# philips/janus

Hardware: AMD Instinct MI355X
Metric: reports prepared+aggregated/sec (helper, Prio3Histogram len=256) at 1/2/4/8 GPUs (higher is better)
Workload: dtype u32 limbs (Field128 mod-p integer arithmetic); 1 GPU; Prio3Histogram length=256 chunk_length=16 helper prepare_init+prepare_shares_to_prepare_message+prepare_next+aggregate, 1 segment; reports_per_gpu=1048576, global_batch=1048576, parallelism=dp1 (report shards; RCCL all-gather + mod-p combine)

## Files before the change

### include/janus_prio3.h

```cpp
#ifndef JANUS_PRIO3_H
#define JANUS_PRIO3_H
#include <stddef.h>
#include <stdint.h>

#ifdef __cplusplus
extern "C" {
#endif

enum {
  PRIO3_COUNT = 0,
  PRIO3_SUM = 1,
  PRIO3_SUMVEC = 2,
  PRIO3_HISTOGRAM = 3,
  PRIO3_SUMVEC_F64_MP = 4,
  PRIO3_FPVEC_BOUNDED_L2 = 5,
};

enum {
  PRIO3_STATUS_FINISHED = 0,
  PRIO3_STATUS_PREP_INIT = 1,
  PRIO3_STATUS_PREP_SHARE_DECODE = 2,
  PRIO3_STATUS_PREP_MSG = 3,
  PRIO3_STATUS_PREP_NEXT = 4,
  PRIO3_STATUS_PEER_MISMATCH = 5,
// ... 170 lines not shown
                             uint8_t* status);

struct janus_hpke_sealer;
int prio3_client_report_stride(const prio3_params* params,
                               const struct janus_hpke_sealer* leader_sealer,
                               const struct janus_hpke_sealer* helper_sealer,
                               int with_taskprov_extension);
int prio3_client_prepare_reports_device(
    prio3_engine* engine, struct janus_hpke_sealer* leader_sealer,
    struct janus_hpke_sealer* helper_sealer, uint32_t n, const uint8_t task_id[32],
    uint64_t time_precision, const uint64_t* d_measurements, const uint8_t* d_report_ids,
    const uint64_t* d_times, const uint8_t* d_rand, const uint8_t* d_sk_e_leader,
    const uint8_t* d_sk_e_helper, uint8_t leader_config_id, uint8_t helper_config_id,
    int with_taskprov_extension, uint8_t* d_reports, uint32_t report_stride,
    uint32_t* d_report_len, uint8_t* d_status, void* stream);

int prio3_client_generate_device(prio3_engine* engine, uint32_t n, uint64_t seed,
                                 uint64_t first_index, uint8_t* d_nonces,
                                 uint8_t* d_public_shares, uint8_t* d_helper_shares,
                                 uint8_t* d_leader_prep_shares, uint64_t* d_measurements,
                                 uint8_t* d_leader_out_shares, uint8_t* d_flags,
                                 uint8_t* d_leader_input_shares, void* stream);

int prio3_device_trim(int device);

int prio3_engine_set_option(prio3_engine* engine, const char* key, int64_t value);
int prio3_engine_timing(prio3_engine* engine, char* names, size_t names_cap, double* ms,
                        uint64_t* launches, int cap);
void prio3_engine_timing_reset(prio3_engine* engine);
int prio3_trace_enabled(void);

int prio3_selftest_field(int op, uint32_t n, const uint8_t* a, const uint8_t* b, uint8_t* out);

#ifdef __cplusplus
}
#endif
#endif
```

### janus_amd/csrc/prio3_device.h

```cpp
#pragma once
#include <hip/hip_runtime.h>
#include <stdint.h>

#define DEV __device__ __forceinline__
#ifndef F128_ASM
#define F128_ASM 1
#endif

struct f128 {
  uint32_t w[4];
};

DEV f128 mk128(uint32_t a, uint32_t b, uint32_t c, uint32_t d) {
  f128 r;
  r.w[0] = a;
  r.w[1] = b;
  r.w[2] = c;
  r.w[3] = d;
  return r;
}
DEV f128 zero128() { return mk128(0, 0, 0, 0); }
DEV f128 sel128(bool c, const f128& a, const f128& b) {
  return mk128(c ? a.w[0] : b.w[0], c ? a.w[1] : b.w[1], c ? a.w[2] : b.w[2], c ? a.w[3] : b.w[3]);
}
// ... 639 lines not shown
#pragma unroll
  for (int i = 0; i < N / 2; i++) {
    const uint32_t lo = v[i], hi = v[i + N / 2];
    const uint32_t send = sel ? lo : hi, keep = sel ? hi : lo;
    v[i] = keep + (uint32_t)__builtin_amdgcn_update_dpp(0, (int)send, CTRL, 0xf, 0xf, false);
  }
}
DEV uint32_t wave_halfsum2(const f128& x0, const f128& x1, uint32_t lane) {
  uint32_t v[16];
#pragma unroll
  for (int w = 0; w < 4; w++) {
    v[2 * w] = x0.w[w] & 0xffffu;
    v[2 * w + 1] = x0.w[w] >> 16;
    v[8 + 2 * w] = x1.w[w] & 0xffffu;
    v[8 + 2 * w + 1] = x1.w[w] >> 16;
  }
#pragma unroll
  for (int i = 0; i < 8; i++) {
    const auto r = __builtin_amdgcn_permlane32_swap(v[i], v[i + 8], false, false);
    v[i] = r[0] + r[1];
  }
#pragma unroll
  for (int i = 0; i < 4; i++) {
    const auto r = __builtin_amdgcn_permlane16_swap(v[i], v[i + 4], false, false);
    v[i] = r[0] + r[1];
  }
  halfsum_stage<4, 0x140, 3>(v, lane);
  halfsum_stage<2, 0x141, 2>(v, lane);
  uint32_t x = v[0];
  x += (uint32_t)__builtin_amdgcn_update_dpp(0, (int)x, 0xB1, 0xf, 0xf, false);
  x += (uint32_t)__builtin_amdgcn_update_dpp(0, (int)x, 0x4E, 0xf, 0xf, false);
  return x;
}
```

### janus_amd/csrc/prio3_engine.hip

```cpp
#include <hip/hip_runtime.h>

#include <cstdio>
#include <cstdlib>
#include <cstring>
#include <functional>
#include <mutex>
#include <string>
#include <thread>
#include <type_traits>
#include <vector>

#include "../../include/janus_hpke.h"
#include "../../include/janus_prio3.h"
#include "prio3_device.h"

#include "prio3_common.h"
#include "prio3_query_sum.h"
#include "prio3_runtime.h"
#include "sha256_device.h"
#include "sha256_host.h"

#ifndef XOFD_OCC
#define XOFD_OCC 3
#endif
template <class F>
__device__ __forceinline__ void xof_body(const DevParams& p, const InPtrs& in, const Scratch& sc,
                                         const uint32_t r) {
  if (r >= p.n) return;
  constexpr uint32_t ES = F::ES;
  uint32_t flag = p.force_slow;
  uint32_t nonce[4], km[4], kp[4], kb[4] = {0, 0, 0, 0};
  load16(in.nonces + 16 * (size_t)r, nonce);
  const uint8_t* hs = in.helper + (size_t)r * p.helper_share_len;
  load16(hs, km);
  load16(hs + 16, kp);
  const bool JR = p.jr_len > 0;
  if (JR) load16(hs + 32, kb);

  {
    KState s;
    kzero(s);
    Msg m;
    msg_zero(m);
    msg_dst(m, p.dst[5]);
    {
      uint32_t vk[4];
      load_vk(p, in, r, vk);
      msg_bytes16(m, 9, vk);
    }
    msg_byte(m, 25, 1);
    msg_bytes16(m, 26, nonce);
    msg_absorb_final(s, m, 42);
    uint32_t q0 = 0, q1 = 0;
    squeeze_block<F>(p, s, 0, p.qr_len, q0, q1, sc.qr, r, flag);
// ... 168 lines not shown
    msg_dst(m, p.dst[5]);
    {
      uint32_t vk[4];
      load_vk(p, in, r, vk);
      msg_bytes16(m, 9, vk);
    }
    msg_byte(m, 25, 1);
    msg_bytes16(m, 26, nonce);
    msg_absorb_final(s, m, 42);
    if (p.qr_len == 1) {
      uint32_t w[4] = {kword(s, 0), kword(s, 1), kword(s, 2), kword(s, 3)};
      put_elem<F>(p, sc.qr, 0, r, w, flag);
    } else {
      uint32_t q0 = 0, q1 = 0;
      squeeze_block<F>(p, s, 0, p.qr_len, q0, q1, sc.qr, r, flag);
    }
  }
  const uint32_t M = p.meas_len, K = (M * 16 + 167) / 168;
  const uint32_t L = 42 + M * 16, B = L / 168, rem = L % 168;
  KState ms, js;
  kzero(ms);
  kzero(js);
  {
    Msg m;
    msg_zero(m);
    msg_dst(m, p.dst[1]);
    msg_bytes16(m, 9, km);
    msg_byte(m, 25, 1);
    msg_absorb_final(ms, m, 26);
  }
  uint32_t pend0 = 0, pend1 = 0;
  TruncSink ts(p, sc.out, r);
  const int Mi = (int)M;
  auto fused_pair = [&](int e0, f128 a, f128 b2) __attribute__((always_inline)) {
    if (e0 >= Mi) return;
    if (haspad && oor) {
      a = zero128();
      b2 = zero128();
    }
    const uint32_t tot = wave_halfsum2(a, b2, lane);
    const int e = e0 + (int)(lane >> 5);
    if ((lane & 3u) == 0 && e < Mi)
      sc.wpart[((size_t)(r >> 6) * M + (uint32_t)e) * 8u + ((lane >> 2) & 7u)] = tot;
  };
  auto fuse_block = [&](uint32_t b, uint32_t q0, uint32_t q1) __attribute__((always_inline)) {
    const int e0 = 21 * (int)(b >> 1);
    const f128 z = zero128();
    if ((b & 1) == 0) {
#pragma unroll
      for (int t = 0; t < 10; t += 2)
        fused_pair(e0 + t, mk128(kword(ms, 4 * t), kword(ms, 4 * t + 1), kword(ms, 4 * t + 2),
                                 kword(ms, 4 * t + 3)),
                   mk128(kword(ms, 4 * t + 4), kword(ms, 4 * t + 5), kword(ms, 4 * t + 6),
                         kword(ms, 4 * t + 7)));
    } else {
      fused_pair(e0 + 10, mk128(q0, q1, kword(ms, 0), kword(ms, 1)),
                 mk128(kword(ms, 2), kword(ms, 3), kword(ms, 4), kword(ms, 5)));
#pragma unroll
      for (int t = 1; t < 10; t += 2)
        fused_pair(e0 + 11 + t,
                   mk128(kword(ms, 2 + 4 * t), kword(ms, 3 + 4 * t), kword(ms, 4 + 4 * t),
                         kword(ms, 5 + 4 * t)),
                   t + 1 < 10 ? mk128(kword(ms, 6 + 4 * t), kword(ms, 7 + 4 * t),
                                      kword(ms, 8 + 4 * t), kword(ms, 9 + 4 * t))
                              : z);
    }
  };
  auto wmask = [&](int j) __attribute__((always_inline)) {
    const uint32_t lo = 4u * (uint32_t)j;
    return (lo + 4 <= rem) ? 0xffffffffu : (lo >= rem ? 0u : ((1u << (8 * (rem - lo))) - 1u));
  };
  auto carry_tail = [&](bool last) __attribute__((always_inline)) {
#pragma unroll
    for (int j = 0; j < 10; j++) {
      uint32_t x = __builtin_amdgcn_alignbit(kword(ms, 32 + j), kword(ms, 31 + j), 16);
      if (last) x &= wmask(j);
      kxor_word(js, j, x);
    }
    uint32_t x = kword(ms, 41) >> 16;
    if (last) x &= wmask(10);
    kxor_word(js, 10, x);
  };
  {
    if (FUSE && fuse) fuse_block(0, 0, 0);
    squeeze_meas<TR>(p, ms, 0, M, pend0, pend1, sc.meas, r, flag, ts);
    Msg m;
    msg_zero(m);
    msg_dst(m, p.dst[7]);
    msg_bytes16(m, 9, kb);
    msg_byte(m, 25, 1);
    msg_bytes16(m, 26, nonce);
#pragma unroll
    for (int j = 0; j < 10; j++) kxor_word(js, j, m.w[j]);
    kxor_word(js, 10, (m.w[10] & 0xffffu) | (kword(ms, 0) << 16));
#pragma unroll
    for (int j = 11; j < 42; j++)
      kxor_word(js, j, __builtin_amdgcn_alignbit(kword(ms, j - 10), kword(ms, j - 11), 16));
    keccak_p12(js);
    carry_tail(B == 1);
    keccak_p12(ms);
  }
  if constexpr (PULL) {
    if (in.seg_dst) in.seg_dst[r] = in.seg_src[r];
    if (in.accept_dst) in.accept_dst[r] = in.accept_src[r];
  }
  const uint32_t Q = PULL ? p.prep_share_len / 16 : 0u;
  const size_t wbase = PULL ? (size_t)(r - lane) * (p.prep_share_len / 16) + lane : 0;
  const uint4* lsrc = PULL ? (const uint4*)in.leader_src + wbase : nullptr;
  uint4* ldst = PULL ? (uint4*)in.leader + wbase : nullptr;
#pragma unroll 1
  for (uint32_t b = 1; b < B; b++) {
    uint4 pc0, pc1;
    uint32_t q0 = 0, q1 = 0;
    if constexpr (PULL) {
      q0 = Q * (b - 1) / (B - 1);
      q1 = Q * b / (B - 1);
      if (q0 < q1) pc0 = lsrc[64 * (size_t)q0];
      if (q0 + 1 < q1) pc1 = lsrc[64 * (size_t)(q0 + 1)];
    }
    if (FUSE && fuse) fuse_block(b, pend0, pend1);
    squeeze_meas<TR>(p, ms, b, M, pend0, pend1, sc.meas, r, flag, ts);
    kxor_word(js, 10, kword(ms, 0) << 16);
#pragma unroll
    for (int j = 11; j < 42; j++)
      kxor_word(js, j, __builtin_amdgcn_alignbit(kword(ms, j - 10), kword(ms, j - 11), 16));
    keccak_p12(js);
    carry_tail(b + 1 == B);
    if (b + 1 < K) keccak_p12(ms);
    if constexpr (PULL) {
      if (q0 < q1) ldst[64 * (size_t)q0] = pc0;
      if (q0 + 1 < q1) ldst[64 * (size_t)(q0 + 1)] = pc1;
    }
  }
  uint32_t part[4];
  {
    const bool hasW = B < K;
    if (FUSE && fuse && hasW) fuse_block(B, pend0, pend1);
    if (hasW) squeeze_meas<TR>(p, ms, B, M, pend0, pend1, sc.meas, r, flag, ts);
#pragma unroll
    for (int j = 0; j < 42; j++) {
      uint32_t x = 0;
      if (j == 10) x = hasW ? kword(ms, 0) << 16 : 0u;
      else if (j > 10)
        x = hasW ? __builtin_amdgcn_alignbit(kword(ms, j - 10), kword(ms, j - 11), 16) : 0u;
      x &= wmask(j);
      if ((uint32_t)j == (rem >> 2)) x ^= 1u << (8 * (rem & 3));
      if (j == 41) x ^= 0x80000000u;
      kxor_word(js, j, x);
    }
    keccak_p12(js);
    part[0] = kword(js, 0);
    part[1] = kword(js, 1);
    part[2] = kword(js, 2);
    part[3] = kword(js, 3);
  }
  {
    uint32_t kp[4];
    load16(hs + 16, kp);
    KState s;
    kzero(s);
    Msg m;
    msg_zero(m);
    msg_dst(m, p.dst[2]);
    msg_bytes16(m, 9, kp);
    msg_byte(m, 25, 1);
    msg_byte(m, 26, 1);
    msg_absorb_final(s, m, 27);
    const uint32_t PL = p.proof_len, Kp = (PL * 16 + 167) / 168;
    uint32_t q0 = 0, q1 = 0;
    for (uint32_t b = 0; b < Kp; b++) {
      squeeze_block<F>(p, s, b, PL, q0, q1, sc.proofs, r, flag);
      if (b + 1 < Kp) keccak_p12(s);
    }
  }
  {
    uint32_t pub0[4];
    load16(in.pub + (size_t)r * p.public_share_len, pub0);
    KState s;
    kzero(s);
    Msg m;
    msg_zero(m);
    msg_dst(m, p.dst[6]);
    msg_bytes16(m, 25, pub0);
    msg_bytes16(m, 41, part);
    msg_absorb_final(s, m, 57);
    uint32_t cor[4] = {kword(s, 0), kword(s, 1), kword(s, 2), kword(s, 3)};
    KState t;
    kzero(t);
    Msg m2;
    msg_zero(m2);
    msg_dst(m2, p.dst[3]);
    msg_bytes16(m2, 9, cor);
    msg_byte(m2, 25, 1);
    msg_absorb_final(t, m2, 26);
    uint32_t q0 = 0, q1 = 0;
    squeeze_block<F>(p, t, 0, p.jr_len, q0, q1, sc.jr, r, flag);
    sc.part[r] = make_uint4(part[0], part[1], part[2], part[3]);
    sc.corrected[r] = make_uint4(cor[0], cor[1], cor[2], cor[3]);
  }
  sc.flag[r] = (uint8_t)flag;
  if constexpr (FUSE) {
    if (fuse) {
      const bool anyflag = __any(flag != 0);
      if (lane == 0) sc.wseg[r >> 6] = anyflag ? 0xffffffffu : s0;
    }
  }
}
template <bool FUSE, bool TR = false>
__global__ __launch_bounds__(256, XOFD_OCC) void k_xofd(DevParams p, InPtrs in, Scratch sc) {
  xofd_body<FUSE, TR>(p, in, sc, blockIdx.x * blockDim.x + threadIdx.x);
}

struct ZeroRanges {
  uint8_t* dst[4];
  size_t bytes[4];
};
__global__ __launch_bounds__(256) void k_zero(ZeroRanges z) {
  const size_t tid = blockIdx.x * (size_t)blockDim.x + threadIdx.x, nth = (size_t)gridDim.x * blockDim.x;
#pragma unroll
  for (int k = 0; k < 4; k++) {
    uint8_t* d = z.dst[k];
    const size_t n = z.bytes[k];
    if (!d || !n) continue;
    const size_t head = std::min(n, (size_t)((16 - ((uintptr_t)d & 15)) & 15));
    const size_t n16 = (n - head) / 16;
    for (size_t i = tid; i < n16; i += nth) ((uint4*)(d + head))[i] = make_uint4(0, 0, 0, 0);
    for (size_t i = tid * 4; i < head; i += nth * 4) *(uint32_t*)(d + i) = 0u;
    for (size_t i = head + 16 * n16 + tid * 4; i < n; i += nth * 4) *(uint32_t*)(d + i) = 0u;
  }
}

struct PullRanges {
  const uint8_t* src[4];
  uint8_t* dst[4];
  size_t bytes[4];
};
DEV void pull_body(const PullRanges& pr, size_t tid, size_t nth) {
#pragma unroll
  for (int k = 0; k < 4; k++) {
    const size_t n16 = pr.bytes[k] / 16;
    const uint4* s16 = (const uint4*)pr.src[k];
    uint4* d16 = (uint4*)pr.dst[k];
// ... 1175 lines not shown
  const T PT = F::add(lv(A + 1), pt);
  if (status == PRIO3_STATUS_FINISHED) {
    if (!decode_ok)
      status = PRIO3_STATUS_PREP_SHARE_DECODE;
    else if (!F::is_zero(V0) || !F::eq(G, PT))
      status = PRIO3_STATUS_PREP_MSG;
  }
  uint32_t lpart[4], msg[4];
  load16(lps + (size_t)p.verifier_len * F::ES, lpart);
  if (!prep_msg_check(p, in, sc, r, lpart, msg) && status == PRIO3_STATUS_FINISHED)
    status = PRIO3_STATUS_PREP_NEXT;
  if (status != PRIO3_STATUS_FINISHED) msg[0] = msg[1] = msg[2] = msg[3] = 0;
  ((uint4*)out.prep_msgs)[r] = make_uint4(msg[0], msg[1], msg[2], msg[3]);
  out.status[r] = status;
  }
  if (p.kind == PRIO3_SUMVEC) {
    for (uint32_t e = 0; e < p.out_len; e++) {
      T acc = F::zero(), pw = F::one();
      for (uint32_t b = 0; b < p.bits; b++) {
        acc = F::add(acc, F::mul(pw, ldf<F>(sc.meas, e * p.bits + b, ld, r)));
        pw = F::add(pw, pw);
      }
      F::store(sc.out, (size_t)e * ld + r, acc);
    }
  }
}
template <int GS, int PP, int LEADER = 0>
__global__ __launch_bounds__(256, 3) void k_query_h(DevParams p, InPtrs in, Scratch sc,
                                                  OutPtrs out) {
  query_h_body<GS, PP, LEADER>(p, in, sc, out, blockIdx.x * blockDim.x + threadIdx.x);
}

template <bool FUSE, bool PULL = false>
__global__ __launch_bounds__(256, 3) void k_prep_h(DevParams p, InPtrs in, Scratch sc,
                                                   OutPtrs out) {
  const uint32_t r = blockIdx.x * blockDim.x + threadIdx.x;
  xofd_body<FUSE, false, PULL>(p, in, sc, r);
  query_h_body<2, 32>(p, in, sc, out, r);
}

template <int PP>
__global__ __launch_bounds__(256, 3) void k_leader_prep(DevParams p, InPtrs in, Scratch sc,
                                                        OutPtrs out, uint32_t* wpart,
                                                        uint32_t* wseg) {
  const uint32_t r = blockIdx.x * blockDim.x + threadIdx.x;
  leader_jr_body(p, in, sc, out.status, wpart, wseg, r);
  query_h_body<2, PP, 1>(p, in, sc, out, r);
}

template <int NPH>
__global__ __launch_bounds__(256, 3) void k_prep_sum(DevParams p, InPtrs in, Scratch sc,
                                                     OutPtrs out) {
  const uint32_t r = blockIdx.x * blockDim.x + threadIdx.x;
  xofd_body<false, false>(p, in, sc, r);
  qsum::query_sum_body<NPH, 0>(p, in, sc, out, r);
}





template <class F, int SG>
__global__ __launch_bounds__(256) void k_acc_seg(uint32_t n, size_t ld, uint32_t chunk,
                                                 uint32_t out_len, uint32_t nseg, const void* src,
                                                 const uint8_t* status, const uint32_t* seg,
                                                 const uint8_t* accept, void* partial,
                                                 uint64_t* pcount) {
// ... 534 lines not shown
    iv_out[2 * s] = hi ? lo : 0;
    iv_out[2 * s + 1] = hi ? hi - lo : 0;
  }
}

__global__ void k_meta_final(uint32_t n_segments, unsigned long long* iv) {
  const uint32_t s = blockIdx.x * blockDim.x + threadIdx.x;
  if (s >= n_segments) return;
  const unsigned long long lo = iv[2 * s], hi = iv[2 * s + 1];
  iv[2 * s] = hi ? lo : 0;
  iv[2 * s + 1] = hi ? hi - lo : 0;
}


__global__ void k_selftest_f128(int op, uint32_t n, const uint4* a, const uint4* b, uint4* out) {
  const uint32_t i = blockIdx.x * blockDim.x + threadIdx.x;
  if (i >= n) return;
  auto ld = [](const uint4* p, size_t k) {
    const uint4 v = p[k];
    return mk128(v.x, v.y, v.z, v.w);
  };
  f128 z;
  if (op == 0) z = mul128(ld(a, i), ld(b, i));
  else if (op == 1) z = mul128_asm(ld(a, i), ld(b, i));
  else if (op == 2) z = add128(ld(a, i), ld(b, i));
  else if (op == 3) z = sub128(ld(a, i), ld(b, i));
  else {
    mac128 m;
    mac_zero(m);
    for (int k = 0; k < 16; k++) mac_add(m, ld(a, (size_t)i * 16 + k), ld(b, (size_t)i * 16 + k));
    z = op == 4 ? mac_reduce(m) : mac_reduce_asm(m);
  }
  out[i] = make_uint4(z.w[0], z.w[1], z.w[2], z.w[3]);
}




struct prio3_batch {
  prio3_engine* e;
  Run* run;
  uint32_t c0, n;
};

static uint32_t next_pow2(uint32_t n) {
  uint32_t p = 1;
  while (p < n) p <<= 1;
  return p;
}

static uint32_t optimal_chunk_length(uint32_t m) {
  if (m <= 1) return 1;
  uint32_t max_log2 = 0;
  while ((1u << max_log2) < m) max_log2++;
  max_log2 += 1;
  uint64_t best = UINT64_MAX;
  uint32_t best_chunk = 1;
  for (uint32_t l = max_log2; l >= 1; l--) {
    const uint64_t calls = (1ull << l) - 1, chunk = (m + calls - 1) / calls;
    const uint64_t cost = 2 * chunk + 2 * ((1ull << l) - 1) + 1;
    if (cost < best) {
      best = cost;
      best_chunk = (uint32_t)chunk;
    }
  }
  return best_chunk;
// ... 531 lines not shown
  const bool dual = dp.es == 16 && dp.jr_len && (42 + dp.meas_len * 16) / 168 >= 2;
  if (dp.kind == PRIO3_SUM) return dual && !fuse && query_sum_takes(dp);
  return ps && dual && dp.P == 32;
}

enum : int { DEFER_NONE = 0, DEFER_QH = 1, DEFER_SUM = 2, DEFER_GEN64 = 3 };
static int launch_prepare(prio3_engine* e, const DevParams& base, uint32_t c0, uint32_t n,
                          InPtrs in, OutPtrs out, Scratch sc, hipStream_t st, bool fuse,
                          int* deferred, bool pair = false) {
  DevParams dp = base;
  dp.n = n;
  dp.force_slow = (uint32_t)e->force_slow;
  dp.slow_defer = 0;
  dp.redo = 0;
  const size_t es = dp.es;
  in.nonces += 16 * (size_t)c0;
  if (in.pub) in.pub += (size_t)dp.public_share_len * c0;
  in.helper += (size_t)dp.helper_share_len * c0;
  in.leader += (size_t)dp.prep_share_len * c0;
  if (in.vk_slot) in.vk_slot += c0;
  out.prep_msgs += (size_t)(dp.kind == PRIO3_SUMVEC_F64_MP ? 32 : 16) * c0;
  out.status += c0;
  void** soa[] = {&sc.meas, &sc.proofs, &sc.jr, &sc.qr, &sc.Lbuf, &sc.PVbuf, &sc.acc, &sc.out,
                  &sc.beta};
  for (auto q : soa)
    if (*q) *q = (uint8_t*)*q + es * c0;
  sc.part += c0;
  sc.corrected += c0;
  sc.flag += c0;
  if (sc.seg) sc.seg += c0;
  if (sc.wseg) sc.wseg += c0 / 64;
  if (sc.wpart) sc.wpart += (size_t)(c0 / 64) * dp.meas_len * 8;
  const uint32_t blocks = (n + 255) / 256;
  if (dp.kind == PRIO3_SUMVEC_F64_MP) {
    int rc = PRIO3_OK;
    TIMED(e, st, "k_mp64_prepare", (rc = launch_mp64(e, n, dp.ld, in, out, sc, st)));
    return rc;
  }
  if (dp.kind == PRIO3_FPVEC_BOUNDED_L2) {
    uint32_t nsub, sub;
    const bool qwide = !e->force_generic && fpvec_query_wide_takes(dp);
    fp_sub_sizes(e, n, dp.ld, qwide, nsub, sub);
    for (uint32_t si = 0; si < nsub; si++) {
      const uint32_t s0 = si * sub;
      DevParams q = dp;
      q.n = si + 1 < nsub ? sub : n - s0;
      InPtrs qi = in;
      qi.nonces += 16 * (size_t)s0;
      qi.pub += (size_t)dp.public_share_len * s0;
      qi.helper += (size_t)dp.helper_share_len * s0;
      qi.leader += (size_t)dp.prep_share_len * s0;
      if (qi.vk_slot) qi.vk_slot += s0;
      OutPtrs qo = out;
      qo.prep_msgs += 16 * (size_t)s0;
      qo.status += s0;
      Scratch qs = sc;
      qs.out = (uint8_t*)sc.out + es * s0;
      const uint32_t qb = (q.n + 255) / 256;
      const bool dual = (42 + dp.meas_len * 16) / 168 >= 2;
      q.trunc_xof = dual ? 1u : 0u;
      bool paired = false;
      if (dual) TIMED(e, st, "k_xof_pair", (paired = launch_xof_pair(q, qi, qs, st)));
      if (!paired && dual)
        TIMED(e, st, "k_xofd", (k_xofd<false, true><<<qb, 256, 0, st>>>(q, qi, qs)));
      else if (!paired)
        TIMED(e, st, "k_xof", (k_xof<Fp128><<<qb, 256, 0, st>>>(q, qi, qs)));
      TIMED(e, st, "k_xof_slow", launch_xof_slow<Fp128>(e, q, qi, qs, st));
      if (qwide)
        TIMED(e, st, "k_query_fpw", launch_fpvec_query(q, qi, qs, qo, st, true, false));
      else
        TIMED(e, st, "k_query_fp", launch_fpvec_query(q, qi, qs, qo, st, false, false));
    }
    return PRIO3_OK;
  }
  if (dp.es == 16) {
    const bool ps = dp.kind == PRIO3_HISTOGRAM || dp.kind == PRIO3_SUMVEC;
    const bool wide = ps && !e->force_generic && dp.P != 32 && query_wide_takes(dp);
    const bool dual = dp.jr_len && (42 + dp.meas_len * 16) / 168 >= 2;
    dp.trunc_xof = dp.kind == PRIO3_SUMVEC && wide && dual && !fuse ? 1u : 0u;
    if (prep_fused_takes(e, dp, fuse)) {
      dp.slow_defer = 1u;
      if (dp.kind == PRIO3_SUM) {
        if (deferred) *deferred = DEFER_SUM;
        switch (dp.P) {
          case 16: TIMED(e, st, "k_prep_sum", (k_prep_sum<1><<<blocks, 256, 0, st>>>(dp, in, sc, out))); break;
          case 32: TIMED(e, st, "k_prep_sum", (k_prep_sum<2><<<blocks, 256, 0, st>>>(dp, in, sc, out))); break;
          case 64: TIMED(e, st, "k_prep_sum", (k_prep_sum<4><<<blocks, 256, 0, st>>>(dp, in, sc, out))); break;
          default: TIMED(e, st, "k_prep_sum", (k_prep_sum<8><<<blocks, 256, 0, st>>>(dp, in, sc, out))); break;
        }
      } else {
        if (deferred) *deferred = DEFER_QH;
        const bool pl = in.leader_src != nullptr;
        bool paired = false;
        if (pair)
          TIMED(e, st, "k_prep_hp", (paired = launch_prep_pair(dp, in, sc, out, st, fuse, pl)));
        if (paired) {
        } else if (fuse && pl)
          TIMED(e, st, "k_prep_h", (k_prep_h<true, true><<<blocks, 256, 0, st>>>(dp, in, sc, out)));
        else if (fuse)
          TIMED(e, st, "k_prep_h", (k_prep_h<true><<<blocks, 256, 0, st>>>(dp, in, sc, out)));
        else if (pl)
          TIMED(e, st, "k_prep_h", (k_prep_h<false, true><<<blocks, 256, 0, st>>>(dp, in, sc, out)));
        else
          TIMED(e, st, "k_prep_h", (k_prep_h<false><<<blocks, 256, 0, st>>>(dp, in, sc, out)));
      }
      return PRIO3_OK;
    }
    if (dual) {
      if (fuse)
        TIMED(e, st, "k_xofd", (k_xofd<true><<<blocks, 256, 0, st>>>(dp, in, sc)));
      else if (dp.trunc_xof)
        TIMED(e, st, "k_xofd", (k_xofd<false, true><<<blocks, 256, 0, st>>>(dp, in, sc)));
      else
        TIMED(e, st, "k_xofd", (k_xofd<false><<<blocks, 256, 0, st>>>(dp, in, sc)));
    } else {
      TIMED(e, st, "k_xof_a", (k_xof_a<Fp128><<<blocks, 256, 0, st>>>(dp, in, sc)));
      TIMED(e, st, "k_jrpart", (k_jrpart<false><<<blocks, 256, 0, st>>>(dp, in, sc)));
    }
    const bool qh_path =
        ps && !e->force_generic && !wide && (dp.P == 32 || dp.P == 16 || dp.P == 8);
    dp.slow_defer = qh_path ? 1u : 0u;
    if (qh_path && deferred) *deferred = DEFER_QH;
    if (!qh_path) TIMED(e, st, "k_xof_slow", launch_xof_slow<Fp128>(e, dp, in, sc, st));
    bool done = false;
    if (wide) TIMED(e, st, "k_query_w", (done = launch_query_wide(dp, in, sc, out, st)));
    if (done) {
    } else if (qh_path && dp.P == 32)
      TIMED(e, st, "k_query_h", (k_query_h<2, 32><<<blocks, 256, 0, st>>>(dp, in, sc, out)));
    else if (qh_path && dp.P == 16)
      TIMED(e, st, "k_query_h", (k_query_h<2, 16><<<blocks, 256, 0, st>>>(dp, in, sc, out)));
    else if (qh_path && dp.P == 8)
      TIMED(e, st, "k_query_h", (k_query_h<2, 8><<<blocks, 256, 0, st>>>(dp, in, sc, out)));
    else if (ps)
      TIMED(e, st, "k_query_ps", (k_query_ps<4><<<blocks, 256, 0, st>>>(dp, in, sc, out)));
    else {
      bool qs = false;
      if (!e->force_generic && query_sum_takes(dp))
        TIMED(e, st, "k_query_sum", (qs = launch_query_sum(dp, in, sc, out, st)));
      if (!qs) TIMED(e, st, "k_query", (k_query<Fp128><<<blocks, 256, 0, st>>>(dp, in, sc, out)));
    }
  } else {
    dp.slow_defer = 1u;
    if (deferred) *deferred = DEFER_GEN64;
    TIMED(e, st, "k_prep_gen", (k_prep_gen<Fp64><<<blocks, 256, 0, st>>>(dp, in, sc, out)));
  }
  return PRIO3_OK;
}
// ... 1954 lines not shown
    return exec_leader_next(&job);
  }
  int rc = prio3_leader_prepare_next_batch(b, prep_msgs, status_inout);
  if (rc == PRIO3_OK)
    rc = prio3_accumulate(b, segment_ids, accept_mask, n_segments, agg_shares_out, counts_out);
  return rc;
}

int prio3_trace_enabled(void) { return trace_enabled() ? 1 : 0; }

int prio3_selftest_field(int op, uint32_t n, const uint8_t* a, const uint8_t* b, uint8_t* out) {
  if (op < 0 || op > 5) return PRIO3_EINVAL;
  if (n == 0) return PRIO3_OK;
  const size_t m = (op >= 4 ? 16 : 1) * (size_t)n * 16;
  void *da = nullptr, *db = nullptr, *dout = nullptr;
  int rc = PRIO3_OK;
  if (hipMalloc(&da, m) != hipSuccess || hipMalloc(&db, m) != hipSuccess ||
      hipMalloc(&dout, (size_t)n * 16) != hipSuccess ||
      hipMemcpy(da, a, m, hipMemcpyHostToDevice) != hipSuccess ||
      hipMemcpy(db, b, m, hipMemcpyHostToDevice) != hipSuccess) {
    rc = PRIO3_EDEVICE;
  } else {
    k_selftest_f128<<<(n + 255) / 256, 256>>>(op, n, (const uint4*)da, (const uint4*)db, (uint4*)dout);
    if (hipGetLastError() != hipSuccess ||
        hipMemcpy(out, dout, (size_t)n * 16, hipMemcpyDeviceToHost) != hipSuccess)
      rc = PRIO3_EDEVICE;
  }
  (void)hipFree(da);
  (void)hipFree(db);
  (void)hipFree(dout);
  return rc;
}

}
```

### janus_amd/prio3.py

```python
from __future__ import annotations

import ctypes as C
import os
from dataclasses import dataclass
from typing import Optional

import numpy as np

_HERE = os.path.dirname(os.path.abspath(__file__))
LIB_PATH = os.environ.get("JANUS_PRIO3_LIB") or os.path.join(_HERE, "libjanus_prio3.so")

PRIO3_COUNT, PRIO3_SUM, PRIO3_SUMVEC, PRIO3_HISTOGRAM, PRIO3_SUMVEC_F64_MP = 0, 1, 2, 3, 4
PRIO3_FPVEC_BOUNDED_L2 = 5

STATUS_FINISHED = 0
STATUS_PREP_INIT = 1
STATUS_PREP_SHARE_DECODE = 2
STATUS_PREP_MSG = 3
STATUS_PREP_NEXT = 4
STATUS_PEER_MISMATCH = 5
STATUS_INPUT_SHARE_DECODE = 6
STATUS_HPKE_DECRYPT = 0x84
STATUS_INVALID_MESSAGE = 0x88
STATUS_REPORT_TOO_EARLY = 0x89
# ... 28 lines not shown

class Prio3ExecutorStats(C.Structure):
    _fields_ = [(n, C.c_uint64) for n in ("jobs", "reports", "groups", "active_jobs",
                                          "active_reports")]


EXEC_PREPARE, EXEC_ACCUMULATE, EXEC_LEADER_INIT, EXEC_LEADER_NEXT = 0, 1, 2, 3


class Prio3Sizes(C.Structure):
    _fields_ = [(n, C.c_uint32) for n in (
        "field_bytes", "meas_len", "out_len", "proof_len", "verifier_len", "joint_rand_len",
        "nonce_len", "public_share_len", "helper_share_len", "prep_share_len", "prep_msg_len",
        "agg_share_len", "leader_input_share_len")]


EXPORTED_SYMBOLS = (
    "prio3_sizes", "prio3_engine_create", "prio3_engine_destroy", "prio3_helper_prepare_batch",
    "prio3_helper_prepare_aggregate_batch",
    "prio3_accumulate", "prio3_debug_output_shares", "prio3_batch_free", "prio3_device_prepare",
    "prio3_device_accumulate", "prio3_device_output_shares", "prio3_device_combine",
    "prio3_engine_set_option", "prio3_engine_timing", "prio3_engine_timing_reset",
    "prio3_client_generate_device", "prio3_selftest_field", "prio3_trace_enabled", "prio3_device_prepare_aggregate",
    "prio3_device_trim",
    "prio3_device_aggregate_finish", "prio3_leader_prepare_init_batch",
    "prio3_leader_prepare_next_batch", "prio3_device_leader_prepare_init",
    "prio3_device_leader_prepare_next", "prio3_device_batch_metadata", "prio3_batch_metadata",
    "prio3_device_combine_metadata", "prio3_engine_create_ex", "prio3_engine_create_mask",
    "prio3_engine_create_devices", "prio3_engine_members", "prio3_executor_control",
    "prio3_executor_stats_get", "prio3_helper_aggregate_init_batch",
    "prio3_helper_aggregate_init_batch_ex",
    "prio3_leader_prepare_next_aggregate_batch",
    "prio3_client_shard_device", "prio3_client_shard_batch", "prio3_client_prepare_reports_device",
    "prio3_client_rand_len", "prio3_client_report_stride",
)
HPKE_EXPORTED_SYMBOLS = (
    "janus_hpke_opener_create", "janus_hpke_opener_destroy",
    "janus_hpke_open_input_shares_device", "janus_hpke_open_input_shares",
    "janus_hpke_open_device", "janus_hpke_open", "janus_hpke_set_timing", "janus_hpke_timing",
    "janus_hpke_selftest_p256", "janus_hpke_selftest_field", "janus_hpke_executor_stats_get",
    "janus_hpke_executor_control",
    "janus_hpke_sealer_create", "janus_hpke_sealer_destroy", "janus_hpke_seal_device",
    "janus_hpke_seal", "janus_hpke_seal_input_shares_device", "janus_hpke_seal_input_shares",
)

_lib = None


def load_library() -> C.CDLL:
    global _lib
    if _lib is not None:
        return _lib
    if not os.path.exists(LIB_PATH):
        raise ImportError(f"janus_amd HIP engine not built: {LIB_PATH} is missing "
                          "(run `make -C janus_amd` or __graft_entry__.build())")
    try:
        import torch
    except ImportError:
        pass
    L = C.CDLL(LIB_PATH, mode=C.RTLD_GLOBAL)
    P, u8p, vp = C.POINTER, C.POINTER(C.c_uint8), C.c_void_p
    L.prio3_sizes.argtypes = [P(Prio3Params), P(Prio3Sizes)]
    L.prio3_engine_create.argtypes = [P(Prio3Params), u8p, C.c_int, P(vp)]
    L.prio3_engine_create_ex.argtypes = [P(Prio3Params), u8p, C.c_size_t, C.c_int, P(vp)]
    L.prio3_engine_create_mask.argtypes = [P(Prio3Params), u8p, C.c_size_t, C.c_int, P(vp)]
    L.prio3_engine_create_devices.argtypes = [P(Prio3Params), u8p, C.c_size_t, P(C.c_int),
                                              C.c_uint32, P(vp)]
    L.prio3_engine_members.argtypes = [vp, P(Prio3MemberInfo), C.c_uint32]
    L.prio3_executor_control.argtypes = [vp, C.c_int, C.c_char_p, C.c_int64]
    L.prio3_executor_stats_get.argtypes = [vp, C.c_uint32, C.c_int, P(Prio3ExecutorStats)]
    L.prio3_engine_destroy.argtypes = [vp]
    L.prio3_engine_destroy.restype = None
    L.prio3_helper_prepare_batch.argtypes = [vp, C.c_uint32, vp, vp, vp, vp, vp, vp, P(vp)]
    L.prio3_accumulate.argtypes = [vp, vp, vp, C.c_uint32, vp, vp]
    L.prio3_helper_prepare_aggregate_batch.argtypes = [vp, C.c_uint32, vp, vp, vp, vp, vp, vp,
                                                       C.c_uint32, vp, vp, vp, vp]
    u32 = C.c_uint32
    L.prio3_helper_aggregate_init_batch.argtypes = [vp, vp, u32, vp, C.c_int, vp, vp, vp, vp, vp,
                                                    vp, u32, vp, vp, vp, u32, vp, vp, vp, vp]
    L.prio3_helper_aggregate_init_batch_ex.argtypes = [vp, vp, vp, C.c_uint64, u32, vp, C.c_int, vp,
                                                       vp, vp, vp, vp, vp, u32, vp, vp, vp, u32,
                                                       vp, vp, vp, vp]
    L.prio3_debug_output_shares.argtypes = [vp, vp]
    L.prio3_batch_free.argtypes = [vp]
    L.prio3_batch_free.restype = None
    L.prio3_device_prepare.argtypes = [vp, C.c_uint32, vp, vp, vp, vp, vp, vp, vp]
    L.prio3_device_accumulate.argtypes = [vp, C.c_uint32, vp, vp, vp, C.c_uint32, vp, vp, vp]
    L.prio3_device_output_shares.argtypes = [vp, C.c_uint32, vp]
    L.prio3_device_combine.argtypes = [vp, C.c_uint32, C.c_uint32, vp, vp, vp, vp, vp]
    L.prio3_client_generate_device.argtypes = [vp, C.c_uint32, C.c_uint64, C.c_uint64, vp, vp,
                                               vp, vp, vp, vp, vp, vp, vp]
    L.prio3_engine_set_option.argtypes = [vp, C.c_char_p, C.c_int64]
    L.prio3_engine_timing.argtypes = [vp, C.c_char_p, C.c_size_t, P(C.c_double),
                                      P(C.c_uint64), C.c_int]
    L.prio3_engine_timing_reset.argtypes = [vp]
    L.prio3_engine_timing_reset.restype = None
    L.prio3_selftest_field.argtypes = [C.c_int, C.c_uint32, vp, vp, vp]
    L.prio3_trace_enabled.argtypes = []
    L.prio3_device_trim.argtypes = [C.c_int]
    L.prio3_device_prepare_aggregate.argtypes = [vp, C.c_uint32, vp, vp, vp, vp, vp, C.c_uint32,
                                                 vp, vp, vp]
    L.prio3_device_aggregate_finish.argtypes = [vp, vp, vp, vp, vp, vp]
    L.prio3_leader_prepare_init_batch.argtypes = [vp, C.c_uint32, vp, vp, vp, vp, vp, P(vp)]
    L.prio3_leader_prepare_next_batch.argtypes = [vp, vp, vp]
    L.prio3_leader_prepare_next_aggregate_batch.argtypes = [vp, vp, vp, vp, vp, C.c_uint32, vp,
                                                            vp]
    L.prio3_device_leader_prepare_init.argtypes = [vp, C.c_uint32, vp, vp, vp, vp, vp, vp]
    L.prio3_device_leader_prepare_next.argtypes = [vp, C.c_uint32, vp, vp, vp]
    L.prio3_device_batch_metadata.argtypes = [vp, C.c_uint32, vp, vp, vp, vp, vp, C.c_uint32, vp,
                                              vp, vp]
    L.prio3_batch_metadata.argtypes = [vp, C.c_uint32, vp, vp, vp, vp, vp, C.c_uint32, vp, vp]
    L.prio3_device_combine_metadata.argtypes = [vp, C.c_uint32, C.c_uint32, vp, vp, vp, vp, vp]
    L.prio3_client_rand_len.argtypes = [P(Prio3Params)]
    L.prio3_client_shard_device.argtypes = [vp, u32, vp, vp, vp, vp, vp, vp, vp, vp]
    L.prio3_client_shard_batch.argtypes = [vp, u32, vp, vp, vp, vp, vp, vp, vp]
    L.prio3_client_report_stride.argtypes = [P(Prio3Params), vp, vp, C.c_int]
    L.prio3_client_prepare_reports_device.argtypes = [vp, vp, vp, u32, vp, C.c_uint64, vp, vp, vp,
                                                      vp, vp, vp, C.c_uint8, C.c_uint8, C.c_int,
                                                      vp, u32, vp, vp, vp]
    _lib = L
    return L


def trim_device_pool(device: int = 0) -> None:
    rc = load_library().prio3_device_trim(device)
    if rc:
        raise RuntimeError(f"prio3_device_trim failed (rc={rc})")


def selftest_field(op: int, a: np.ndarray, b: np.ndarray) -> np.ndarray:
    a = np.ascontiguousarray(a, np.uint8)
    b = np.ascontiguousarray(b, np.uint8)
    n = a.shape[0] // (16 if op >= 4 else 1)
    out = np.zeros((n, 16), np.uint8)
    rc = load_library().prio3_selftest_field(op, n, _np_ptr(a), _np_ptr(b), _np_ptr(out))
    if rc:
        raise RuntimeError(f"prio3_selftest_field failed (rc={rc})")
    return out


@dataclass(frozen=True)
class Prio3:
    kind: int
    bits: int = 0
    length: int = 0
    chunk_length: int = 0
    num_proofs: int = 1

    def params(self) -> Prio3Params:
        return Prio3Params(self.kind, self.bits, self.length, self.chunk_length, self.num_proofs)

    def sizes(self) -> Prio3Sizes:
        s = Prio3Sizes()
        rc = load_library().prio3_sizes(C.byref(self.params()), C.byref(s))
        if rc:
            raise ValueError(f"unsupported Prio3 parameters (rc={rc})")
        return s


def Prio3Count() -> Prio3:
    return Prio3(PRIO3_COUNT)


def Prio3Sum(bits: int) -> Prio3:
    return Prio3(PRIO3_SUM, bits=bits)


def Prio3SumVec(bits: int, length: int, chunk_length: int) -> Prio3:
    return Prio3(PRIO3_SUMVEC, bits=bits, length=length, chunk_length=chunk_length)

# ... 582 lines not shown
```

Measured before the change: 176.8 million reports/s.

## Stage fused histogram partial sums through LDS tile and defer wave reduction

Measurement field elements squeezed from the XOF are now written into a per-wave shared-memory tile, up to 8 elements at a time. The wave-level half-sum reduction then runs batched after the joint-randomness keccak permutation, replacing the per-pair register permlane reductions that ran inline. The aim is to cut cross-lane shuffle work, spread the reduction across the keccak phases and produce more coalesced partial-sum writes. This adds LDS traffic, wavefront fences and shared memory per block, which may reduce occupancy. The block size also becomes a macro, and a selftest entry point for the tile reduction is added.

Result: faster. 179.0 million reports/s (median of 6 runs) (+1.2%).

```diff
diff --git a/include/janus_prio3.h b/include/janus_prio3.h
--- a/include/janus_prio3.h
+++ b/include/janus_prio3.h
@@ -226,6 +226,8 @@
 
 int prio3_selftest_field(int op, uint32_t n, const uint8_t* a, const uint8_t* b, uint8_t* out);
 
+int prio3_selftest_tile(uint32_t n_elems, const uint8_t* values, uint32_t* out);
+
 #ifdef __cplusplus
 }
 #endif
diff --git a/janus_amd/csrc/prio3_device.h b/janus_amd/csrc/prio3_device.h
--- a/janus_amd/csrc/prio3_device.h
+++ b/janus_amd/csrc/prio3_device.h
@@ -695,3 +695,47 @@
   x += (uint32_t)__builtin_amdgcn_update_dpp(0, (int)x, 0x4E, 0xf, 0xf, false);
   return x;
 }
+
+constexpr int FTILE = 8;
+DEV void tile_fence() {
+  __builtin_amdgcn_fence(__ATOMIC_RELEASE, "wavefront");
+  __builtin_amdgcn_wave_barrier();
+  __builtin_amdgcn_fence(__ATOMIC_ACQUIRE, "wavefront");
+}
+DEV void tile_stage(uint4* tile, int slot, uint32_t lane, const f128& x) {
+  tile[slot * 64 + (int)lane] = make_uint4(x.w[0], x.w[1], x.w[2], x.w[3]);
+}
+DEV uint32_t tile_halfsum(const uint4* tile, uint32_t lane) {
+  const uint32_t j = lane & 7u;
+  const uint4* row = tile + j * 64u + (j ^ (lane >> 3));
+  sum128 s;
+  {
+    const uint4 x = row[0];
+    s.w[0] = x.x, s.w[1] = x.y, s.w[2] = x.z, s.w[3] = x.w, s.w[4] = 0;
+  }
+#pragma unroll
+  for (int i = 1; i < 8; i++) {
+    const uint4 x = row[8 * i];
+    sum_add(s, mk128(x.x, x.y, x.z, x.w));
+  }
+  uint32_t v[8];
+#pragma unroll
+  for (int w = 0; w < 4; w++) {
+    v[2 * w] = s.w[w] & 0xffffu;
+    v[2 * w + 1] = s.w[w] >> 16;
+  }
+  v[7] += s.w[4] << 16;
+#pragma unroll
+  for (int i = 0; i < 4; i++) {
+    const auto r = __builtin_amdgcn_permlane32_swap(v[i], v[i + 4], false, false);
+    v[i] = r[0] + r[1];
+  }
+#pragma unroll
+  for (int i = 0; i < 2; i++) {
+    const auto r = __builtin_amdgcn_permlane16_swap(v[i], v[i + 2], false, false);
+    v[i] = r[0] + r[1];
+  }
+  const bool sel = (lane >> 3) & 1;
+  const uint32_t send = sel ? v[0] : v[1], keep = sel ? v[1] : v[0];
+  return keep + (uint32_t)__builtin_amdgcn_update_dpp(0, (int)send, 0x128, 0xf, 0xf, false);
+}
diff --git a/janus_amd/csrc/prio3_engine.hip b/janus_amd/csrc/prio3_engine.hip
--- a/janus_amd/csrc/prio3_engine.hip
+++ b/janus_amd/csrc/prio3_engine.hip
@@ -20,6 +20,9 @@
 #include "sha256_device.h"
 #include "sha256_host.h"
 
+#ifndef XOFD_BLOCK
+#define XOFD_BLOCK 256
+#endif
 #ifndef XOFD_OCC
 #define XOFD_OCC 3
 #endif
@@ -254,39 +257,62 @@
   uint32_t pend0 = 0, pend1 = 0;
   TruncSink ts(p, sc.out, r);
   const int Mi = (int)M;
-  auto fused_pair = [&](int e0, f128 a, f128 b2) __attribute__((always_inline)) {
-    if (e0 >= Mi) return;
-    if (haspad && oor) {
-      a = zero128();
-      b2 = zero128();
-    }
-    const uint32_t tot = wave_halfsum2(a, b2, lane);
-    const int e = e0 + (int)(lane >> 5);
-    if ((lane & 3u) == 0 && e < Mi)
-      sc.wpart[((size_t)(r >> 6) * M + (uint32_t)e) * 8u + ((lane >> 2) & 7u)] = tot;
+  uint4* tile = nullptr;
+  if constexpr (FUSE) {
+    __shared__ uint4 fuse_tiles[XOFD_BLOCK / 64][FTILE * 64];
+    tile = fuse_tiles[__builtin_amdgcn_readfirstlane(threadIdx.x >> 6)];
+  }
+  uint32_t* const wrow =
+      FUSE && !PULL ? sc.wpart + (size_t)__builtin_amdgcn_readfirstlane(r >> 6) * M * 8u
+                    : nullptr;
+  const uint32_t wlane = (lane & 7u) * 8u + (lane >> 3);
+  auto mword = [&](int w) __attribute__((always_inline)) {
+    return mk128(kword(ms, w), kword(ms, w + 1), kword(ms, w + 2), kword(ms, w + 3));
   };
-  auto fuse_block = [&](uint32_t b, uint32_t q0, uint32_t q1) __attribute__((always_inline)) {
+  auto stage = [&](int e, int slot, f128 x) __attribute__((always_inline)) {
+    if (e >= Mi) return;
+    if (haspad && oor) x = zero128();
+    tile_stage(tile, slot, lane, x);
+  };
+  auto flush = [&](int eb, int n) __attribute__((always_inline)) {
+    const int cnt = min(n, Mi - eb);
+    if (cnt <= 0) return;
+    tile_fence();
+    const uint32_t tot = tile_halfsum(tile, lane);
+    if ((int)(lane & 7u) < cnt) {
+      if constexpr (PULL) sc.wpart[((size_t)(r >> 6) * M + (uint32_t)eb) * 8u + wlane] = tot;
+      else (wrow + (size_t)eb * 8u)[wlane] = tot;
+    }
+    tile_fence();
+  };
+  auto fuse_top = [&](uint32_t b, uint32_t q0, uint32_t q1) __attribute__((always_inline)) {
     const int e0 = 21 * (int)(b >> 1);
-    const f128 z = zero128();
     if ((b & 1) == 0) {
-#pragma unroll
-      for (int t = 0; t < 10; t += 2)
-        fused_pair(e0 + t, mk128(kword(ms, 4 * t), kword(ms, 4 * t + 1), kword(ms, 4 * t + 2),
-                                 kword(ms, 4 * t + 3)),
-                   mk128(kword(ms, 4 * t + 4), kword(ms, 4 * t + 5), kword(ms, 4 * t + 6),
-                         kword(ms, 4 * t + 7)));
+      if (b) flush(e0 - 5, 5);
+#pragma unroll
+      for (int t = 0; t < 8; t++) stage(e0 + t, t, mword(4 * t));
     } else {
-      fused_pair(e0 + 10, mk128(q0, q1, kword(ms, 0), kword(ms, 1)),
-                 mk128(kword(ms, 2), kword(ms, 3), kword(ms, 4), kword(ms, 5)));
-#pragma unroll
-      for (int t = 1; t < 10; t += 2)
-        fused_pair(e0 + 11 + t,
-                   mk128(kword(ms, 2 + 4 * t), kword(ms, 3 + 4 * t), kword(ms, 4 + 4 * t),
-                         kword(ms, 5 + 4 * t)),
-                   t + 1 < 10 ? mk128(kword(ms, 6 + 4 * t), kword(ms, 7 + 4 * t),
-                                      kword(ms, 8 + 4 * t), kword(ms, 9 + 4 * t))
-                              : z);
-    }
+      stage(e0 + 10, 2, mk128(q0, q1, kword(ms, 0), kword(ms, 1)));
+#pragma unroll
+      for (int t = 0; t < 5; t++) stage(e0 + 11 + t, 3 + t, mword(2 + 4 * t));
+    }
+  };
+  auto fuse_mid = [&](uint32_t b) __attribute__((always_inline)) {
+    const int e0 = 21 * (int)(b >> 1);
+    if ((b & 1) == 0) {
+      flush(e0, 8);
+      stage(e0 + 8, 0, mword(32));
+      stage(e0 + 9, 1, mword(36));
+    } else {
+      flush(e0 + 8, 8);
+#pragma unroll
+      for (int t = 0; t < 5; t++) stage(e0 + 16 + t, t, mword(22 + 4 * t));
+    }
+  };
+  auto fuse_tail = [&](uint32_t b) __attribute__((always_inline)) {
+    const int e0 = 21 * (int)(b >> 1);
+    if ((b & 1) == 0) flush(e0 + 8, 2);
+    else flush(e0 + 16, 5);
   };
   auto wmask = [&](int j) __attribute__((always_inline)) {
     const uint32_t lo = 4u * (uint32_t)j;
@@ -304,7 +330,7 @@
     kxor_word(js, 10, x);
   };
   {
-    if (FUSE && fuse) fuse_block(0, 0, 0);
+    if (FUSE && fuse) fuse_top(0, 0, 0);
     squeeze_meas<TR>(p, ms, 0, M, pend0, pend1, sc.meas, r, flag, ts);
     Msg m;
     msg_zero(m);
@@ -319,6 +345,7 @@
     for (int j = 11; j < 42; j++)
       kxor_word(js, j, __builtin_amdgcn_alignbit(kword(ms, j - 10), kword(ms, j - 11), 16));
     keccak_p12(js);
+    if (FUSE && fuse) fuse_mid(0);
     carry_tail(B == 1);
     keccak_p12(ms);
   }
@@ -340,13 +367,14 @@
       if (q0 < q1) pc0 = lsrc[64 * (size_t)q0];
       if (q0 + 1 < q1) pc1 = lsrc[64 * (size_t)(q0 + 1)];
     }
-    if (FUSE && fuse) fuse_block(b, pend0, pend1);
+    if (FUSE && fuse) fuse_top(b, pend0, pend1);
     squeeze_meas<TR>(p, ms, b, M, pend0, pend1, sc.meas, r, flag, ts);
     kxor_word(js, 10, kword(ms, 0) << 16);
 #pragma unroll
     for (int j = 11; j < 42; j++)
       kxor_word(js, j, __builtin_amdgcn_alignbit(kword(ms, j - 10), kword(ms, j - 11), 16));
     keccak_p12(js);
+    if (FUSE && fuse) fuse_mid(b);
     carry_tail(b + 1 == B);
     if (b + 1 < K) keccak_p12(ms);
     if constexpr (PULL) {
@@ -357,7 +385,7 @@
   uint32_t part[4];
   {
     const bool hasW = B < K;
-    if (FUSE && fuse && hasW) fuse_block(B, pend0, pend1);
+    if (FUSE && fuse && hasW) fuse_top(B, pend0, pend1);
     if (hasW) squeeze_meas<TR>(p, ms, B, M, pend0, pend1, sc.meas, r, flag, ts);
 #pragma unroll
     for (int j = 0; j < 42; j++) {
@@ -371,6 +399,10 @@
       kxor_word(js, j, x);
     }
     keccak_p12(js);
+    if (FUSE && fuse) {
+      if (hasW) fuse_mid(B);
+      fuse_tail(hasW ? B : B - 1);
+    }
     part[0] = kword(js, 0);
     part[1] = kword(js, 1);
     part[2] = kword(js, 2);
@@ -429,7 +461,7 @@
   }
 }
 template <bool FUSE, bool TR = false>
-__global__ __launch_bounds__(256, XOFD_OCC) void k_xofd(DevParams p, InPtrs in, Scratch sc) {
+__global__ __launch_bounds__(XOFD_BLOCK, XOFD_OCC) void k_xofd(DevParams p, InPtrs in, Scratch sc) {
   xofd_body<FUSE, TR>(p, in, sc, blockIdx.x * blockDim.x + threadIdx.x);
 }
 
@@ -1671,7 +1703,7 @@
 }
 
 template <bool FUSE, bool PULL = false>
-__global__ __launch_bounds__(256, 3) void k_prep_h(DevParams p, InPtrs in, Scratch sc,
+__global__ __launch_bounds__(XOFD_BLOCK, 3) void k_prep_h(DevParams p, InPtrs in, Scratch sc,
                                                    OutPtrs out) {
   const uint32_t r = blockIdx.x * blockDim.x + threadIdx.x;
   xofd_body<FUSE, false, PULL>(p, in, sc, r);
@@ -2272,6 +2304,20 @@
     z = op == 4 ? mac_reduce(m) : mac_reduce_asm(m);
   }
   out[i] = make_uint4(z.w[0], z.w[1], z.w[2], z.w[3]);
+}
+
+__global__ __launch_bounds__(64) void k_selftest_tile(uint32_t cnt, const uint4* in,
+                                                      uint32_t* out) {
+  __shared__ uint4 tile[FTILE * 64];
+  const uint32_t lane = threadIdx.x;
+#pragma unroll
+  for (int s = 0; s < FTILE; s++) {
+    const uint4 v = in[s * 64 + (int)lane];
+    tile_stage(tile, s, lane, mk128(v.x, v.y, v.z, v.w));
+  }
+  tile_fence();
+  const uint32_t tot = tile_halfsum(tile, lane);
+  if ((lane & 7u) < cnt) out[(lane & 7u) * 8u + (lane >> 3)] = tot;
 }
 
 
@@ -2869,6 +2915,7 @@
   if (sc.wseg) sc.wseg += c0 / 64;
   if (sc.wpart) sc.wpart += (size_t)(c0 / 64) * dp.meas_len * 8;
   const uint32_t blocks = (n + 255) / 256;
+  const uint32_t xblocks = (n + XOFD_BLOCK - 1) / XOFD_BLOCK;
   if (dp.kind == PRIO3_SUMVEC_F64_MP) {
     int rc = PRIO3_OK;
     TIMED(e, st, "k_mp64_prepare", (rc = launch_mp64(e, n, dp.ld, in, out, sc, st)));
@@ -2899,7 +2946,9 @@
       bool paired = false;
       if (dual) TIMED(e, st, "k_xof_pair", (paired = launch_xof_pair(q, qi, qs, st)));
       if (!paired && dual)
-        TIMED(e, st, "k_xofd", (k_xofd<false, true><<<qb, 256, 0, st>>>(q, qi, qs)));
+        TIMED(e, st, "k_xofd",
+              (k_xofd<false, true><<<(q.n + XOFD_BLOCK - 1) / XOFD_BLOCK, XOFD_BLOCK, 0, st>>>(
+                  q, qi, qs)));
       else if (!paired)
         TIMED(e, st, "k_xof", (k_xof<Fp128><<<qb, 256, 0, st>>>(q, qi, qs)));
       TIMED(e, st, "k_xof_slow", launch_xof_slow<Fp128>(e, q, qi, qs, st));
@@ -2933,23 +2982,23 @@
           TIMED(e, st, "k_prep_hp", (paired = launch_prep_pair(dp, in, sc, out, st, fuse, pl)));
         if (paired) {
         } else if (fuse && pl)
-          TIMED(e, st, "k_prep_h", (k_prep_h<true, true><<<blocks, 256, 0, st>>>(dp, in, sc, out)));
+          TIMED(e, st, "k_prep_h", (k_prep_h<true, true><<<xblocks, XOFD_BLOCK, 0, st>>>(dp, in, sc, out)));
         else if (fuse)
-          TIMED(e, st, "k_prep_h", (k_prep_h<true><<<blocks, 256, 0, st>>>(dp, in, sc, out)));
+          TIMED(e, st, "k_prep_h", (k_prep_h<true><<<xblocks, XOFD_BLOCK, 0, st>>>(dp, in, sc, out)));
         else if (pl)
-          TIMED(e, st, "k_prep_h", (k_prep_h<false, true><<<blocks, 256, 0, st>>>(dp, in, sc, out)));
+          TIMED(e, st, "k_prep_h", (k_prep_h<false, true><<<xblocks, XOFD_BLOCK, 0, st>>>(dp, in, sc, out)));
         else
-          TIMED(e, st, "k_prep_h", (k_prep_h<false><<<blocks, 256, 0, st>>>(dp, in, sc, out)));
+          TIMED(e, st, "k_prep_h", (k_prep_h<false><<<xblocks, XOFD_BLOCK, 0, st>>>(dp, in, sc, out)));
       }
       return PRIO3_OK;
     }
     if (dual) {
       if (fuse)
-        TIMED(e, st, "k_xofd", (k_xofd<true><<<blocks, 256, 0, st>>>(dp, in, sc)));
+        TIMED(e, st, "k_xofd", (k_xofd<true><<<xblocks, XOFD_BLOCK, 0, st>>>(dp, in, sc)));
       else if (dp.trunc_xof)
-        TIMED(e, st, "k_xofd", (k_xofd<false, true><<<blocks, 256, 0, st>>>(dp, in, sc)));
+        TIMED(e, st, "k_xofd", (k_xofd<false, true><<<xblocks, XOFD_BLOCK, 0, st>>>(dp, in, sc)));
       else
-        TIMED(e, st, "k_xofd", (k_xofd<false><<<blocks, 256, 0, st>>>(dp, in, sc)));
+        TIMED(e, st, "k_xofd", (k_xofd<false><<<xblocks, XOFD_BLOCK, 0, st>>>(dp, in, sc)));
     } else {
       TIMED(e, st, "k_xof_a", (k_xof_a<Fp128><<<blocks, 256, 0, st>>>(dp, in, sc)));
       TIMED(e, st, "k_jrpart", (k_jrpart<false><<<blocks, 256, 0, st>>>(dp, in, sc)));
@@ -4970,4 +5019,23 @@
   return rc;
 }
 
-}
+int prio3_selftest_tile(uint32_t n_elems, const uint8_t* values, uint32_t* out) {
+  if (n_elems == 0 || n_elems > (uint32_t)FTILE || !values || !out) return PRIO3_EINVAL;
+  const size_t m = (size_t)FTILE * 64 * 16, mo = (size_t)n_elems * 8 * sizeof(uint32_t);
+  void *din = nullptr, *dout = nullptr;
+  int rc = PRIO3_OK;
+  if (hipMalloc(&din, m) != hipSuccess || hipMalloc(&dout, mo) != hipSuccess ||
+      hipMemcpy(din, values, m, hipMemcpyHostToDevice) != hipSuccess) {
+    rc = PRIO3_EDEVICE;
+  } else {
+    k_selftest_tile<<<1, 64>>>(n_elems, (const uint4*)din, (uint32_t*)dout);
+    if (hipGetLastError() != hipSuccess ||
+        hipMemcpy(out, dout, mo, hipMemcpyDeviceToHost) != hipSuccess)
+      rc = PRIO3_EDEVICE;
+  }
+  (void)hipFree(din);
+  (void)hipFree(dout);
+  return rc;
+}
+
+}
diff --git a/janus_amd/prio3.py b/janus_amd/prio3.py
--- a/janus_amd/prio3.py
+++ b/janus_amd/prio3.py
@@ -84,7 +84,7 @@
     "prio3_helper_aggregate_init_batch_ex",
     "prio3_leader_prepare_next_aggregate_batch",
     "prio3_client_shard_device", "prio3_client_shard_batch", "prio3_client_prepare_reports_device",
-    "prio3_client_rand_len", "prio3_client_report_stride",
+    "prio3_client_rand_len", "prio3_client_report_stride", "prio3_selftest_tile",
 )
 HPKE_EXPORTED_SYMBOLS = (
     "janus_hpke_opener_create", "janus_hpke_opener_destroy",
@@ -148,6 +148,7 @@
     L.prio3_engine_timing_reset.argtypes = [vp]
     L.prio3_engine_timing_reset.restype = None
     L.prio3_selftest_field.argtypes = [C.c_int, C.c_uint32, vp, vp, vp]
+    L.prio3_selftest_tile.argtypes = [C.c_uint32, vp, vp]
     L.prio3_trace_enabled.argtypes = []
     L.prio3_device_trim.argtypes = [C.c_int]
     L.prio3_device_prepare_aggregate.argtypes = [vp, C.c_uint32, vp, vp, vp, vp, vp, C.c_uint32,
@@ -188,6 +189,16 @@
     rc = load_library().prio3_selftest_field(op, n, _np_ptr(a), _np_ptr(b), _np_ptr(out))
     if rc:
         raise RuntimeError(f"prio3_selftest_field failed (rc={rc})")
+    return out
+
+
+def selftest_tile(values: np.ndarray, n_elems: int) -> np.ndarray:
+    values = np.ascontiguousarray(values, np.uint8)
+    assert values.shape == (8, 64, 16)
+    out = np.zeros((n_elems, 8), np.uint32)
+    rc = load_library().prio3_selftest_tile(n_elems, _np_ptr(values), _np_ptr(out))
+    if rc:
+        raise RuntimeError(f"prio3_selftest_tile failed (rc={rc})")
     return out
 
 
```
